# Qualcomm-AI-research/fastforward

Hardware: AMD Instinct MI355X
Metric: tokens/sec Llama-3-8B W8A8 quantized fwd; quant/dequant GB/s vs HBM peak (higher is better)
Workload: dtype int8; 1 GPU; llama3-8b shapes, W8 per-channel symmetric + A8 per-tensor asymmetric on the 7 linears x 32 layers (BASELINE.json configs[2] forward), weights re-quantized every step as in the reference; global_batch=8, seq_len=2048, parallelism=dp1 (batch-sharded replicas, no data-path collective), quantizers=448, launch=hipGraph replay

## Files before the change

### fastforward_amd/csrc/ffq_attention.hip

```cpp
#include "ffq_affine.h"
#include "ffq_common.h"
#include "ffq_vec.h"

#include <math.h>
#include <stdlib.h>


namespace ffq {
namespace {

typedef __attribute__((ext_vector_type(8))) __bf16 bf16x8;
typedef __attribute__((ext_vector_type(16))) float f32x16;
typedef __attribute__((ext_vector_type(4))) short s16x4;
typedef __attribute__((ext_vector_type(8))) short s16x8;

constexpr int kD = 128;
constexpr int kKeys = 64;
#ifndef FFQ_ATTN_WAVES
#define FFQ_ATTN_WAVES 8
#endif
constexpr int kWaves = FFQ_ATTN_WAVES;
constexpr int kRowsPerWave = 32;
constexpr int kQBlock = kWaves * kRowsPerWave;
constexpr int kKPitch = 256;
constexpr int kVPitch = 320;
constexpr int kKBytes = kKeys * kKPitch;
constexpr int kVBytes = kKeys * kVPitch;
constexpr int kLdsBytes = 2 * kKBytes + 2 * kVBytes;
constexpr float kDefer = 8.0f;
constexpr int kOPitch = 272;
static_assert(kWaves * kRowsPerWave * kOPitch <= kLdsBytes, "epilogue image must fit the K/V ring");

struct AttnArgs {
  const uint16_t* q;
  const uint16_t* k;
  const uint16_t* v;
  uint16_t* ctx;
  int8_t* codes;
  const float* scale;
  const float* offset;
  int32_t B, S, H, HKV;
  int32_t nqb;
  float c;
  float lo, hi;
  const uint16_t* q_cos;
  const uint16_t* q_sin;
};

__device__ __forceinline__ bf16x8 load_vt(const unsigned char* vbuf, uint32_t lane_off, int imm) {
  typedef s16x4 __attribute__((address_space(3))) * lds_ptr;
  const s16x4 a = __builtin_amdgcn_ds_read_tr16_b64_v4i16((lds_ptr)(vbuf + lane_off + imm));
  const s16x4 b = __builtin_amdgcn_ds_read_tr16_b64_v4i16((lds_ptr)(vbuf + lane_off + imm + 8 * kVPitch));
  const s16x8 ab = __builtin_shufflevector(a, b, 0, 1, 2, 3, 4, 5, 6, 7);
  return __builtin_bit_cast(bf16x8, ab);
}

template <bool CAUSAL>
__global__ __launch_bounds__(kWaves * 64) void attention_fwd_kernel(AttnArgs a) {
  constexpr int QBLOCK = kQBlock;
  constexpr int PASSES = kKeys / (kWaves * 4);

  extern __shared__ __attribute__((aligned(16))) unsigned char smem[];
  const uint32_t tid = threadIdx.x;
  const uint32_t lane = tid & 63, wave = tid >> 6;
  const uint32_t r32 = lane & 31, h = lane >> 5;

  const uint32_t groups = (uint32_t)(a.H / a.HKV);
  uint32_t bid = blockIdx.x;
  const uint32_t kvh = bid % (uint32_t)a.HKV;
  bid /= (uint32_t)a.HKV;
  const uint32_t hg = bid % groups;
  bid /= groups;
  const uint32_t qb = (uint32_t)a.nqb - 1 - bid % (uint32_t)a.nqb;
  const uint32_t b = bid / (uint32_t)a.nqb;
  const uint32_t head = kvh * groups + hg;

  const int32_t q0 = (int32_t)qb * QBLOCK;
  const int32_t qw0 = q0 + (int32_t)wave * kRowsPerWave;
  const bool wave_valid = qw0 < a.S;
  const int32_t q_end = q0 + QBLOCK < a.S ? q0 + QBLOCK : a.S;
  const int32_t ntiles = (CAUSAL ? q_end : a.S) / kKeys;

  const uint32_t srow = tid >> 4, sslot = tid & 15;
  const size_t kv_stride = (size_t)a.HKV * kD;
  const uint16_t* kbase = a.k + ((size_t)b * a.S * a.HKV + kvh) * kD + sslot * 8;
  const uint16_t* vbase = a.v + ((size_t)b * a.S * a.HKV + kvh) * kD + sslot * 8;
  u32x4 sk[PASSES], sv[PASSES];
  auto stage_load = [&](int32_t tile) {
#pragma unroll
    for (int p = 0; p < PASSES; ++p) {
      const size_t row = (size_t)tile * kKeys + srow + kWaves * 4 * p;
      sk[p] = *reinterpret_cast<const u32x4*>(kbase + row * kv_stride);
      sv[p] = *reinterpret_cast<const u32x4*>(vbase + row * kv_stride);
    }
  };
  auto stage_store = [&](int buf) {
#pragma unroll
    for (int p = 0; p < PASSES; ++p) {
      const uint32_t row = srow + kWaves * 4 * p;
      *reinterpret_cast<u32x4*>(smem + buf * kKBytes + row * kKPitch + ((sslot ^ (row & 15)) << 4)) = sk[p];
      *reinterpret_cast<u32x4*>(smem + 2 * kKBytes + buf * kVBytes + row * kVPitch + (sslot << 4)) = sv[p];
    }
  };

  stage_load(0);

  bf16x8 qf[8];
  {
    const uint16_t* qrow = a.q + (((size_t)b * a.S + (size_t)(wave_valid ? qw0 + (int32_t)r32 : 0)) * a.H + head) * kD;
#pragma unroll
    for (int t = 0; t < 8; ++t) {
      u32x4 v = *reinterpret_cast<const u32x4*>(qrow + (2 * t + h) * 8);
      if (!wave_valid) v = u32x4{0, 0, 0, 0};
      qf[t] = __builtin_bit_cast(bf16x8, v);
    }
    if (a.q_cos && wave_valid) {
      const size_t trow = (size_t)(qw0 + (int32_t)r32) * kD;
#pragma unroll
      for (int t = 0; t < 4; ++t) {
        const int c = (2 * t + (int)h) * 8;
        const u32x4 cl = *reinterpret_cast<const u32x4*>(a.q_cos + trow + c), ch = *reinterpret_cast<const u32x4*>(a.q_cos + trow + 64 + c);
        const u32x4 sl = *reinterpret_cast<const u32x4*>(a.q_sin + trow + c), sh = *reinterpret_cast<const u32x4*>(a.q_sin + trow + 64 + c);
        const u32x4 lo = __builtin_bit_cast(u32x4, qf[t]), hi = __builtin_bit_cast(u32x4, qf[t + 4]);
        const uint32_t lw[4] = {lo.x, lo.y, lo.z, lo.w}, hw[4] = {hi.x, hi.y, hi.z, hi.w};
        const uint32_t clw[4] = {cl.x, cl.y, cl.z, cl.w}, chw[4] = {ch.x, ch.y, ch.z, ch.w};
        const uint32_t slw[4] = {sl.x, sl.y, sl.z, sl.w}, shw[4] = {sh.x, sh.y, sh.z, sh.w};
        uint32_t ol[4], oh[4];
#pragma unroll
        for (int w = 0; w < 4; ++w) {
          float r[2][2];
#pragma unroll
          for (int e = 0; e < 2; ++e) {
            auto el = [&](uint32_t word) { return __builtin_bit_cast(float, e ? (word & 0xFFFF0000u) : (word << 16)); };
            const float x1 = el(lw[w]), x2 = el(hw[w]);
            float p = x1 * el(clw[w]), q2 = (-x2) * el(slw[w]), u = x2 * el(chw[w]), d = x1 * el(shw[w]);
            const uint32_t pq = pack2<bf16_t>(p, q2), ud = pack2<bf16_t>(u, d);
            r[0][e] = __builtin_bit_cast(float, pq << 16) + __builtin_bit_cast(float, pq & 0xFFFF0000u);
            r[1][e] = __builtin_bit_cast(float, ud << 16) + __builtin_bit_cast(float, ud & 0xFFFF0000u);
          }
          ol[w] = pack2<bf16_t>(r[0][0], r[0][1]);
          oh[w] = pack2<bf16_t>(r[1][0], r[1][1]);
        }
        qf[t] = __builtin_bit_cast(bf16x8, u32x4{ol[0], ol[1], ol[2], ol[3]});
        qf[t + 4] = __builtin_bit_cast(bf16x8, u32x4{oh[0], oh[1], oh[2], oh[3]});
      }
    }
  }

  f32x16 o[4];
#pragma unroll
  for (int i = 0; i < 4; ++i)
#pragma unroll
    for (int e = 0; e < 16; ++e) o[i][e] = 0.0f;
  float m_run = -1.0e30f, l_run = 0.0f;

  const uint32_t i16 = lane & 15, g16 = lane >> 4;
  const uint32_t vt_lane_off = (4 * (g16 >> 1) + (i16 >> 2)) * kVPitch + (16 * (g16 & 1) + 4 * (i16 & 3)) * 2;

  stage_store(0);
  __syncthreads();

  for (int32_t tile = 0; tile < ntiles; ++tile) {
    const int buf = tile & 1;
    const bool more = tile + 1 < ntiles;
    if (more) stage_load(tile + 1);
    const int32_t kv0 = tile * kKeys;
    const bool active = wave_valid && (!CAUSAL || kv0 <= qw0 + kRowsPerWave - 1);
    if (active) {
      const unsigned char* kbuf = smem + buf * kKBytes;
      const unsigned char* vbuf = smem + 2 * kKBytes + buf * kVBytes;
      f32x16 s[2];
#pragma unroll
      for (int sub = 0; sub < 2; ++sub)
#pragma unroll
        for (int e = 0; e < 16; ++e) s[sub][e] = 0.0f;
      bf16x8 kf[2][8];
#pragma unroll
      for (int t = 0; t < 8; ++t)
#pragma unroll
        for (int sub = 0; sub < 2; ++sub) {
          const uint32_t krow = 32 * sub + r32;
          kf[sub][t] = *reinterpret_cast<const bf16x8*>(kbuf + krow * kKPitch + (((2 * t + h) ^ (krow & 15)) << 4));
        }
#pragma unroll
      for (int t = 0; t < 8; ++t)
#pragma unroll
        for (int sub = 0; sub < 2; ++sub)
          s[sub] = __builtin_amdgcn_mfma_f32_32x32x16_bf16(kf[sub][t], qf[t], s[sub], 0, 0, 0);
      __builtin_amdgcn_sched_group_barrier(0x100, 16, 0);
      __builtin_amdgcn_sched_group_barrier(0x008, 16, 0);
      if (CAUSAL && kv0 + kKeys - 1 > qw0) {
        const int32_t qi = qw0 + (int32_t)r32;
#pragma unroll
        for (int sub = 0; sub < 2; ++sub)
#pragma unroll
          for (int e = 0; e < 16; ++e) {
            const int32_t key = kv0 + 32 * sub + (e & 3) + 8 * (e >> 2) + 4 * (int32_t)h;
            if (key > qi) s[sub][e] = -INFINITY;
          }
      }
      float mx = s[0][0];
#pragma unroll
      for (int sub = 0; sub < 2; ++sub)
#pragma unroll
        for (int e = 0; e < 16; ++e) mx = fmaxf(mx, s[sub][e]);
      mx = fmaxf(mx, __shfl_xor(mx, 32));
      const float mxs = mx * a.c;
      if (!__all(mxs - m_run <= kDefer)) {
        const float m_new = mxs - m_run > kDefer ? mxs : m_run;
        const float alpha = __builtin_amdgcn_exp2f(m_run - m_new);
        m_run = m_new;
        l_run *= alpha;
#pragma unroll
        for (int i = 0; i < 4; ++i)
#pragma unroll
          for (int e = 0; e < 16; ++e) o[i][e] *= alpha;
      }
      float rs = 0.0f;
      bf16x8 pf[2][2];
#pragma unroll
      for (int sub = 0; sub < 2; ++sub)
#pragma unroll
        for (int e = 0; e < 16; ++e) {
          const float p = __builtin_amdgcn_exp2f(__builtin_fmaf(s[sub][e], a.c, -m_run));
          rs += p;
          pf[sub][e >> 3][e & 7] = (__bf16)p;
        }
      l_run += rs;
#pragma unroll
      for (int db = 0; db < 4; ++db)
#pragma unroll
        for (int sub = 0; sub < 2; ++sub)
#pragma unroll
          for (int u = 0; u < 2; ++u) {
            const int imm = (32 * sub + 16 * u) * kVPitch + 32 * db * 2;
            const bf16x8 vf = load_vt(vbuf, vt_lane_off, imm);
            o[db] = __builtin_amdgcn_mfma_f32_32x32x16_bf16(vf, pf[sub][u], o[db], 0, 0, 0);
          }
    }
    if (more) stage_store(buf ^ 1);
    __syncthreads();
  }

  const float l_tot = l_run + __shfl_xor(l_run, 32);
  const float inv = 1.0f / l_tot;
  unsigned char* obuf = smem + wave * (kRowsPerWave * kOPitch);
#pragma unroll
  for (int db = 0; db < 4; ++db)
#pragma unroll
    for (int rr = 0; rr < 4; ++rr) {
      u32x2 w;
      w.x = pack2<bf16_t>(o[db][4 * rr + 0] * inv, o[db][4 * rr + 1] * inv);
      w.y = pack2<bf16_t>(o[db][4 * rr + 2] * inv, o[db][4 * rr + 3] * inv);
      *reinterpret_cast<u32x2*>(obuf + r32 * kOPitch + (32 * db + 8 * rr + 4 * h) * 2) = w;
    }
  __syncthreads();
  if (!wave_valid) return;
  float sc = 1.0f, of = 0.0f;
  if (a.codes) {
    sc = a.scale[0];
    of = a.offset ? rne(a.offset[0]) : 0.0f;
  }
#pragma unroll
  for (int it = 0; it < 4; ++it) {
    const uint32_t slot = it * 64 + lane;
    const uint32_t row = slot >> 3, seg = slot & 7;
    Chunk<bf16_t, 16> z;
    z.load(reinterpret_cast<const bf16_t*>(obuf + row * kOPitch + seg * 32));
    const size_t at = (((size_t)b * a.S + (size_t)(qw0 + (int32_t)row)) * a.H + head) * kD + seg * 16;
    if (a.ctx) z.store(reinterpret_cast<bf16_t*>(a.ctx) + at);
    if (a.codes) {
      float x[16];
#pragma unroll
      for (int i = 0; i < 16; ++i) x[i] = z.get(i);
      Chunk<int8_t, 16> y;
      quantize_chunk_to_bytes<16>(x, sc, of, a.lo, a.hi, y);
      y.store(a.codes + at);
    }
  }
}

}
}

using namespace ffq;

extern "C" int ffq_attention(const void* q, const void* k, const void* v, int dt, int64_t batch, int64_t seq_len,
                             int64_t q_heads, int64_t kv_heads, int64_t head_dim, double softmax_scale, int causal,
                             void* ctx_out, int8_t* codes_out, const float* out_scale, const float* out_offset,
                             double out_num_bits, const void* q_cos, const void* q_sin, void* stream) {
  hipStream_t s = static_cast<hipStream_t>(stream);
  if (batch < 0 || seq_len < 0 || q_heads <= 0 || kv_heads <= 0) return fail(FFQ_ERR_ARG, "bad extent");
  if (dt != FFQ_BF16) return fail(FFQ_ERR_DTYPE, "attention is built for bf16 activations");
  if (head_dim != kD) return fail(FFQ_ERR_DTYPE, "attention is built for head_dim 128");
  if (seq_len % kKeys != 0) return fail(FFQ_ERR_DTYPE, "attention needs seq_len %% 64 == 0");
  if (q_heads % kv_heads != 0) return fail(FFQ_ERR_ARG, "q_heads must be a multiple of kv_heads");
  if (batch == 0 || seq_len == 0) return FFQ_OK;
  if (!q || !k || !v || (!ctx_out && !codes_out)) return fail(FFQ_ERR_ARG, "NULL buffer");
  if (codes_out && !out_scale) return fail(FFQ_ERR_ARG, "codes need a scale");
  if (codes_out && !(out_num_bits >= 1.0 && out_num_bits <= 8.0 && out_num_bits == (double)(int)out_num_bits))
    return fail(FFQ_ERR_ARG, "codes need an integral bit-width in 1..8");
  if (!aligned16(q) || !aligned16(k) || !aligned16(v) || (ctx_out && !aligned16(ctx_out)) || (codes_out && !aligned16(codes_out)))
    return fail(FFQ_ERR_ARG, "buffers must be 16-byte aligned");
  if (batch * seq_len * q_heads * head_dim >= ((int64_t)1 << 40)) return fail(FFQ_ERR_ARG, "too many elements for one launch");
  if ((q_cos == nullptr) != (q_sin == nullptr)) return fail(FFQ_ERR_ARG, "q_cos and q_sin come together");
  if (q_cos && (!aligned16(q_cos) || !aligned16(q_sin))) return fail(FFQ_ERR_ARG, "buffers must be 16-byte aligned");
  AttnArgs a;
  a.q_cos = static_cast<const uint16_t*>(q_cos); a.q_sin = static_cast<const uint16_t*>(q_sin);
  a.q = static_cast<const uint16_t*>(q); a.k = static_cast<const uint16_t*>(k); a.v = static_cast<const uint16_t*>(v);
  a.ctx = static_cast<uint16_t*>(ctx_out); a.codes = codes_out; a.scale = out_scale; a.offset = out_offset;
  a.B = (int32_t)batch; a.S = (int32_t)seq_len; a.H = (int32_t)q_heads; a.HKV = (int32_t)kv_heads;
  a.nqb = (int32_t)((seq_len + kQBlock - 1) / kQBlock);
  a.c = (float)(softmax_scale * 1.4426950408889634);
  const double half = ldexp(1.0, (int)out_num_bits - 1);
  a.lo = codes_out ? (float)-half : 0.0f;
  a.hi = codes_out ? (float)(half - 1.0) : 0.0f;
  const int64_t blocks = (int64_t)a.nqb * q_heads * batch;
  if (blocks >= ((int64_t)1 << 31)) return fail(FFQ_ERR_ARG, "too many workgroups");
  static uint64_t once_causal = 0, once_full = 0;
  if (causal) ensure_dynamic_lds(&once_causal, reinterpret_cast<const void*>(attention_fwd_kernel<true>), kLdsBytes);
  else ensure_dynamic_lds(&once_full, reinterpret_cast<const void*>(attention_fwd_kernel<false>), kLdsBytes);
  const dim3 grid((unsigned)blocks), block(kWaves * 64);
  if (causal) attention_fwd_kernel<true><<<grid, block, kLdsBytes, s>>>(a);
  else attention_fwd_kernel<false><<<grid, block, kLdsBytes, s>>>(a);
  return check_launch("attention_fwd_kernel");
}
```

### fastforward_amd/csrc/ffq_common.h

```cpp
#pragma once

#include <hip/hip_runtime.h>
#include <stdarg.h>
#include <stdint.h>
#include <stdio.h>

#include "../../include/ffq.h"

#ifndef FFQ_TICKET_ORDER
#define FFQ_TICKET_ORDER __ATOMIC_RELAXED
#endif
#define ffq_ticket_acquire()                                                      \
  do {                                                                            \
    if (FFQ_TICKET_ORDER != __ATOMIC_RELAXED) __builtin_amdgcn_fence(__ATOMIC_ACQUIRE, "agent"); \
  } while (0)

namespace ffq {

char* err_buf();
int fail(int code, const char* fmt, ...);
bool generic_kernels_forced();
bool mid_register_form_forced();
bool splitk_abandon_forced();
bool ring3_form_forced();
bool two_slot_form_forced();
int check_launch(const char* what);

__host__ __device__ inline bool dt_valid(int dt) { return dt >= FFQ_F32 && dt <= FFQ_U8; }
__host__ __device__ inline bool dt_is_float(int dt) {
  return dt == FFQ_F32 || dt == FFQ_BF16 || dt == FFQ_F16 || dt == FFQ_F64;
}
__host__ __device__ inline int dt_size(int dt) {
  switch (dt) {
    case FFQ_F32: case FFQ_I32: return 4;
    case FFQ_BF16: case FFQ_F16: case FFQ_I16: return 2;
    case FFQ_F64: case FFQ_I64: return 8;
    default: return 1;
  }
}

__host__ __device__ inline float bf16_bits_to_f32(uint16_t h) {
  return __builtin_bit_cast(float, (uint32_t)h << 16);
}
__host__ __device__ inline uint16_t f32_to_bf16_bits(float f) {
  uint32_t u = __builtin_bit_cast(uint32_t, f);
  if (f != f) return 0x7FC0;
  u += 0x7FFFu + ((u >> 16) & 1u);
  return (uint16_t)(u >> 16);
}
__host__ __device__ inline float f16_bits_to_f32(uint16_t h) {
  return (float)__builtin_bit_cast(_Float16, h);
}
__host__ __device__ inline uint16_t f32_to_f16_bits(float f) {
  return __builtin_bit_cast(uint16_t, (_Float16)f);
}

__host__ __device__ inline float round_stage(float v, int dt) {
  if (dt == FFQ_BF16) return bf16_bits_to_f32(f32_to_bf16_bits(v));
  if (dt == FFQ_F16) return f16_bits_to_f32(f32_to_f16_bits(v));
  return v;
}

__host__ __device__ inline float rne(float v) { return __builtin_rintf(v); }
__host__ __device__ inline double rne(double v) { return __builtin_rint(v); }

__host__ __device__ inline float clamp_nan(float v, float lo, float hi) {
  float c = v < lo ? lo : v;
  c = c > hi ? hi : c;
  return v != v ? v : c;
}
__host__ __device__ inline double clamp_nan(double v, double lo, double hi) {
  double c = v < lo ? lo : v;
  c = c > hi ? hi : c;
  return v != v ? v : c;
}

__device__ inline double load_any(const void* p, int dt, int64_t i) {
  switch (dt) {
    case FFQ_F32: return (double)((const float*)p)[i];
    case FFQ_BF16: return (double)bf16_bits_to_f32(((const uint16_t*)p)[i]);
    case FFQ_F16: return (double)f16_bits_to_f32(((const uint16_t*)p)[i]);
    case FFQ_F64: return ((const double*)p)[i];
    case FFQ_I8: return (double)((const int8_t*)p)[i];
    case FFQ_I16: return (double)((const int16_t*)p)[i];
    case FFQ_I32: return (double)((const int32_t*)p)[i];
    case FFQ_I64: return (double)((const int64_t*)p)[i];
    default: return (double)((const uint8_t*)p)[i];
  }
}
__device__ inline void store_any(void* p, int dt, int64_t i, double v) {
  const bool nan = v != v;
  switch (dt) {
    case FFQ_F32: ((float*)p)[i] = (float)v; break;
    case FFQ_BF16: ((uint16_t*)p)[i] = f32_to_bf16_bits((float)v); break;
    case FFQ_F16: ((uint16_t*)p)[i] = f32_to_f16_bits((float)v); break;
    case FFQ_F64: ((double*)p)[i] = v; break;
    case FFQ_I8: ((int8_t*)p)[i] = nan ? 0 : (int8_t)(int64_t)v; break;
    case FFQ_I16: ((int16_t*)p)[i] = nan ? 0 : (int16_t)(int64_t)v; break;
    case FFQ_I32: ((int32_t*)p)[i] = nan ? INT32_MIN : (int32_t)(int64_t)v; break;
    case FFQ_I64: ((int64_t*)p)[i] = nan ? INT64_MIN : (int64_t)v; break;
    default: ((uint8_t*)p)[i] = nan ? 0 : (uint8_t)(int64_t)v; break;
  }
}

struct FastDiv {
  uint32_t mul;
  uint32_t shift;
  uint32_t div;
// ... 103 lines not shown
```

### fastforward_amd/csrc/ffq_core.hip

```cpp
#include "ffq_common.h"

#include <math.h>
#include <string.h>

namespace ffq {

static thread_local char g_err[512];

char* err_buf() { return g_err; }

int fail(int code, const char* fmt, ...) {
  va_list ap;
  va_start(ap, fmt);
  vsnprintf(g_err, sizeof g_err, fmt, ap);
  va_end(ap);
  return code;
}

int check_launch(const char* what) {
  hipError_t e = hipGetLastError();
  if (e != hipSuccess) return fail(FFQ_ERR_LAUNCH, "%s: %s", what, hipGetErrorString(e));
  return FFQ_OK;
}

// ... 87 lines not shown
              "The size of tensor a (%lld) must match the size of tensor b (%lld) at non-singleton "
              "dimension 0 (%s vs number of tiles)",
              (long long)ntiles, (long long)numel, what);
}

GenericTiling make_generic(const ffq_tiling* t) {
  GenericTiling g;
  memset(&g, 0, sizeof g);
  g.ndim = t->ndim;
  int64_t s = 1;
  for (int k = t->ndim - 1; k >= 0; --k) {
    g.shape[k] = t->shape[k];
    g.tile[k] = t->tile[k];
    g.gstride[k] = s;
    s *= t->shape[k] / t->tile[k];
  }
  return g;
}

}

using namespace ffq;

extern "C" {

int ffq_abi_version(void) { return FFQ_ABI_VERSION; }
const char* ffq_last_error(void) { return err_buf(); }
const char* ffq_backend_name(void) { return "hip:gfx950"; }

int64_t ffq_num_tiles(const ffq_tiling* tiling) {
  TileInfo info;
  int rc = analyse(tiling, &info);
  if (rc) return -rc;
  return info.ntiles;
}

int ffq_promote_types(int a, int b) {
  if (!dt_valid(a) || !dt_valid(b)) return -FFQ_ERR_ARG;
  if (a == b) return a;
  const bool fa = dt_is_float(a), fb = dt_is_float(b);
  if (fa && !fb) return a;
  if (fb && !fa) return b;
  if (fa && fb) {
    if (a == FFQ_F64 || b == FFQ_F64) return FFQ_F64;
    return FFQ_F32;
  }
  if (a == FFQ_I64 || b == FFQ_I64) return FFQ_I64;
  if (a == FFQ_I32 || b == FFQ_I32) return FFQ_I32;
  return FFQ_I16;
}

int ffq_can_support_bitwidth(int dtype, double num_bits) {
  double avail;
  switch (dtype) {
    case FFQ_BF16: avail = 7; break;
    case FFQ_F16: avail = 10; break;
    case FFQ_F32: avail = 23; break;
    case FFQ_F64: avail = 52; break;
    case FFQ_I8: case FFQ_U8: avail = 8; break;
    case FFQ_I16: avail = 16; break;
    case FFQ_I32: avail = 32; break;
    case FFQ_I64: avail = 64; break;
    default: return 0;
  }
  return (avail + 2) >= num_bits;
}

int ffq_dequantize_result_dtype(int data_dt, int scale_dt, int offset_dt, int has_offset) {
  const int off_dt = has_offset ? offset_dt : scale_dt;
  const int add_dt = ffq_promote_types(data_dt, off_dt);
  if (add_dt < 0) return add_dt;
  return ffq_promote_types(add_dt, scale_dt);
}

}

namespace ffq {
static int g_force_generic = 0;
bool generic_kernels_forced() { return (__atomic_load_n(&g_force_generic, __ATOMIC_RELAXED) & 1) != 0; }
bool splitk_abandon_forced() { return (__atomic_load_n(&g_force_generic, __ATOMIC_RELAXED) & 2) != 0; }
bool mid_register_form_forced() { return (__atomic_load_n(&g_force_generic, __ATOMIC_RELAXED) & 4) != 0; }
bool ring3_form_forced() { return (__atomic_load_n(&g_force_generic, __ATOMIC_RELAXED) & 8) != 0; }
bool two_slot_form_forced() { return (__atomic_load_n(&g_force_generic, __ATOMIC_RELAXED) & 16) != 0; }
}

extern "C" int ffq_force_generic_kernels(int on) {
  return __atomic_exchange_n(&ffq::g_force_generic, on & 31, __ATOMIC_RELAXED);
}
```

Baseline: 139,700 tokens/s.

## Replace per-block attention grid with persistent sorted work walk and GQA head packing

Attention now launches a persistent grid capped at 256 workgroups. Each workgroup walks a list of (batch, kv-head, head-group, row-block) items sorted by causal length and alternates direction on odd rounds, with an XCD-preserving mapping. When the GQA group size is 2, 4 or 8, the heads sharing one KV head are packed into a single item so K/V tiles are loaded once for several query heads. The next item's K/V and Q loads overlap the epilogue of the current one. The aim is to reduce causal tail imbalance and K/V refetch, at the cost of more complex scheduling and extra barriers; the old block form stays available behind a force flag.

```diff
diff --git a/fastforward_amd/csrc/ffq_attention.hip b/fastforward_amd/csrc/ffq_attention.hip
--- a/fastforward_amd/csrc/ffq_attention.hip
+++ b/fastforward_amd/csrc/ffq_attention.hip
@@ -1,4 +1,5 @@
 #include "ffq_affine.h"
+#include "ffq_attn_walk.h"
 #include "ffq_common.h"
 #include "ffq_vec.h"
 
@@ -19,9 +20,13 @@
 #ifndef FFQ_ATTN_WAVES
 #define FFQ_ATTN_WAVES 8
 #endif
+#ifndef FFQ_ATTN_PACK
+#define FFQ_ATTN_PACK 1
+#endif
 constexpr int kWaves = FFQ_ATTN_WAVES;
+constexpr int kAttnWalkWorkgroups = 256;
+static_assert(kWaves * 32 == kWalkBlockRows && 64 == kWalkKeys, "ffq_attn_walk.h describes 8 waves of 32 rows and 64-key tiles");
 constexpr int kRowsPerWave = 32;
-constexpr int kQBlock = kWaves * kRowsPerWave;
 constexpr int kKPitch = 256;
 constexpr int kVPitch = 320;
 constexpr int kKBytes = kKeys * kKPitch;
@@ -40,7 +45,6 @@
   const float* scale;
   const float* offset;
   int32_t B, S, H, HKV;
-  int32_t nqb;
   float c;
   float lo, hi;
   const uint16_t* q_cos;
@@ -55,219 +59,230 @@
   return __builtin_bit_cast(bf16x8, ab);
 }
 
+
+struct Lane {
+  uint32_t lane, wave, r32, h;
+  uint32_t srow, sslot;
+  uint32_t vt_lane_off;
+};
+
+__device__ __forceinline__ Lane make_lane(uint32_t tid, uint32_t wave) {
+  Lane ln;
+  ln.lane = tid & 63; ln.wave = wave;
+  ln.r32 = ln.lane & 31; ln.h = ln.lane >> 5;
+  ln.srow = tid >> 4; ln.sslot = tid & 15;
+  const uint32_t i16 = ln.lane & 15, g16 = ln.lane >> 4;
+  ln.vt_lane_off = (4 * (g16 >> 1) + (i16 >> 2)) * kVPitch + (16 * (g16 & 1) + 4 * (i16 & 3)) * 2;
+  return ln;
+}
+
+constexpr int kPasses = kKeys / (kWaves * 4);
+struct Stage {
+  u32x4 sk[kPasses], sv[kPasses];
+};
+
+
+__device__ __forceinline__ size_t kv_base(const AttnArgs& a, uint32_t b, uint32_t kvh) { return ((size_t)b * a.S * a.HKV + kvh) * kD; }
+
+__device__ __forceinline__ void stage_load(Stage& st, const AttnArgs& a, const Lane& ln, size_t base, int32_t tile) {
+  const uint32_t kv_stride = (uint32_t)a.HKV * kD;
+  const uint32_t lane_off = ln.srow * kv_stride + ln.sslot * 8;
+#pragma unroll
+  for (int p = 0; p < kPasses; ++p) {
+    const size_t rows = base + ((size_t)tile * kKeys + kWaves * 4 * p) * kv_stride;
+    st.sk[p] = *reinterpret_cast<const u32x4*>(a.k + rows + lane_off);
+    st.sv[p] = *reinterpret_cast<const u32x4*>(a.v + rows + lane_off);
+  }
+}
+
+__device__ __forceinline__ void stage_store(const Stage& st, unsigned char* smem, const Lane& ln, int buf) {
+#pragma unroll
+  for (int p = 0; p < kPasses; ++p) {
+    const uint32_t row = ln.srow + kWaves * 4 * p;
+    *reinterpret_cast<u32x4*>(smem + buf * kKBytes + row * kKPitch + ((ln.sslot ^ (row & 15)) << 4)) = st.sk[p];
+    *reinterpret_cast<u32x4*>(smem + 2 * kKBytes + buf * kVBytes + row * kVPitch + (ln.sslot << 4)) = st.sv[p];
+  }
+}
+
+__device__ __forceinline__ void load_q(const AttnArgs& a, const Lane& ln, uint32_t b, uint32_t head, int32_t qw0, bool wave_valid, bf16x8 (&qf)[8]) {
+  if (wave_valid) {
+    const uint16_t* qrows = a.q + (((size_t)b * a.S + (size_t)qw0) * a.H + head) * kD;
+    const uint32_t lane_off = ln.r32 * ((uint32_t)a.H * kD) + ln.h * 8;
+#pragma unroll
+    for (int t = 0; t < 8; ++t) qf[t] = __builtin_bit_cast(bf16x8, *reinterpret_cast<const u32x4*>(qrows + lane_off + 16 * t));
+  } else {
+#pragma unroll
+    for (int t = 0; t < 8; ++t) qf[t] = __builtin_bit_cast(bf16x8, u32x4{0, 0, 0, 0});
+  }
+}
+
+__device__ __forceinline__ void rotate_q(const AttnArgs& a, const Lane& ln, int32_t qw0, bf16x8 (&qf)[8]) {
+  const uint16_t* cos0 = a.q_cos + (size_t)qw0 * kD;
+  const uint16_t* sin0 = a.q_sin + (size_t)qw0 * kD;
+  const uint32_t lane_off = ln.r32 * kD + ln.h * 8;
+  u32x4 tcl[4], tch[4], tsl[4], tsh[4];
+#pragma unroll
+  for (int t = 0; t < 4; ++t) {
+    const uint32_t c = lane_off + 16 * t;
+    tcl[t] = *reinterpret_cast<const u32x4*>(cos0 + c); tch[t] = *reinterpret_cast<const u32x4*>(cos0 + c + 64);
+    tsl[t] = *reinterpret_cast<const u32x4*>(sin0 + c); tsh[t] = *reinterpret_cast<const u32x4*>(sin0 + c + 64);
+  }
+#pragma unroll
+  for (int t = 0; t < 4; ++t) {
+    const u32x4 cl = tcl[t], ch = tch[t], sl = tsl[t], sh = tsh[t];
+    const u32x4 lo = __builtin_bit_cast(u32x4, qf[t]), hi = __builtin_bit_cast(u32x4, qf[t + 4]);
+    const uint32_t lw[4] = {lo.x, lo.y, lo.z, lo.w}, hw[4] = {hi.x, hi.y, hi.z, hi.w};
+    const uint32_t clw[4] = {cl.x, cl.y, cl.z, cl.w}, chw[4] = {ch.x, ch.y, ch.z, ch.w};
+    const uint32_t slw[4] = {sl.x, sl.y, sl.z, sl.w}, shw[4] = {sh.x, sh.y, sh.z, sh.w};
+    uint32_t ol[4], oh[4];
+#pragma unroll
+    for (int w = 0; w < 4; ++w) {
+      float r[2][2];
+#pragma unroll
+      for (int e = 0; e < 2; ++e) {
+        auto el = [&](uint32_t word) { return __builtin_bit_cast(float, e ? (word & 0xFFFF0000u) : (word << 16)); };
+        const float x1 = el(lw[w]), x2 = el(hw[w]);
+        float p = x1 * el(clw[w]), q2 = (-x2) * el(slw[w]), u = x2 * el(chw[w]), d = x1 * el(shw[w]);
+        const uint32_t pq = pack2<bf16_t>(p, q2), ud = pack2<bf16_t>(u, d);
+        r[0][e] = __builtin_bit_cast(float, pq << 16) + __builtin_bit_cast(float, pq & 0xFFFF0000u);
+        r[1][e] = __builtin_bit_cast(float, ud << 16) + __builtin_bit_cast(float, ud & 0xFFFF0000u);
+      }
+      ol[w] = pack2<bf16_t>(r[0][0], r[0][1]);
+      oh[w] = pack2<bf16_t>(r[1][0], r[1][1]);
+    }
+    qf[t] = __builtin_bit_cast(bf16x8, u32x4{ol[0], ol[1], ol[2], ol[3]});
+    qf[t + 4] = __builtin_bit_cast(bf16x8, u32x4{oh[0], oh[1], oh[2], oh[3]});
+  }
+}
+
+struct RowState {
+  f32x16 o[4];
+  float m_run, l_run;
+};
+
+__device__ __forceinline__ void reset_rows(RowState& rs) {
+#pragma unroll
+  for (int i = 0; i < 4; ++i)
+#pragma unroll
+    for (int e = 0; e < 16; ++e) rs.o[i][e] = 0.0f;
+  rs.m_run = -1.0e30f;
+  rs.l_run = 0.0f;
+}
+
 template <bool CAUSAL>
-__global__ __launch_bounds__(kWaves * 64) void attention_fwd_kernel(AttnArgs a) {
-  constexpr int QBLOCK = kQBlock;
-  constexpr int PASSES = kKeys / (kWaves * 4);
-
-  extern __shared__ __attribute__((aligned(16))) unsigned char smem[];
-  const uint32_t tid = threadIdx.x;
-  const uint32_t lane = tid & 63, wave = tid >> 6;
-  const uint32_t r32 = lane & 31, h = lane >> 5;
-
-  const uint32_t groups = (uint32_t)(a.H / a.HKV);
-  uint32_t bid = blockIdx.x;
-  const uint32_t kvh = bid % (uint32_t)a.HKV;
-  bid /= (uint32_t)a.HKV;
-  const uint32_t hg = bid % groups;
-  bid /= groups;
-  const uint32_t qb = (uint32_t)a.nqb - 1 - bid % (uint32_t)a.nqb;
-  const uint32_t b = bid / (uint32_t)a.nqb;
-  const uint32_t head = kvh * groups + hg;
-
-  const int32_t q0 = (int32_t)qb * QBLOCK;
-  const int32_t qw0 = q0 + (int32_t)wave * kRowsPerWave;
-  const bool wave_valid = qw0 < a.S;
-  const int32_t q_end = q0 + QBLOCK < a.S ? q0 + QBLOCK : a.S;
-  const int32_t ntiles = (CAUSAL ? q_end : a.S) / kKeys;
-
-  const uint32_t srow = tid >> 4, sslot = tid & 15;
-  const size_t kv_stride = (size_t)a.HKV * kD;
-  const uint16_t* kbase = a.k + ((size_t)b * a.S * a.HKV + kvh) * kD + sslot * 8;
-  const uint16_t* vbase = a.v + ((size_t)b * a.S * a.HKV + kvh) * kD + sslot * 8;
-  u32x4 sk[PASSES], sv[PASSES];
-  auto stage_load = [&](int32_t tile) {
-#pragma unroll
-    for (int p = 0; p < PASSES; ++p) {
-      const size_t row = (size_t)tile * kKeys + srow + kWaves * 4 * p;
-      sk[p] = *reinterpret_cast<const u32x4*>(kbase + row * kv_stride);
-      sv[p] = *reinterpret_cast<const u32x4*>(vbase + row * kv_stride);
-    }
-  };
-  auto stage_store = [&](int buf) {
-#pragma unroll
-    for (int p = 0; p < PASSES; ++p) {
-      const uint32_t row = srow + kWaves * 4 * p;
-      *reinterpret_cast<u32x4*>(smem + buf * kKBytes + row * kKPitch + ((sslot ^ (row & 15)) << 4)) = sk[p];
-      *reinterpret_cast<u32x4*>(smem + 2 * kKBytes + buf * kVBytes + row * kVPitch + (sslot << 4)) = sv[p];
-    }
-  };
-
-  stage_load(0);
-
-  bf16x8 qf[8];
-  {
-    const uint16_t* qrow = a.q + (((size_t)b * a.S + (size_t)(wave_valid ? qw0 + (int32_t)r32 : 0)) * a.H + head) * kD;
-#pragma unroll
-    for (int t = 0; t < 8; ++t) {
-      u32x4 v = *reinterpret_cast<const u32x4*>(qrow + (2 * t + h) * 8);
-      if (!wave_valid) v = u32x4{0, 0, 0, 0};
-      qf[t] = __builtin_bit_cast(bf16x8, v);
-    }
-    if (a.q_cos && wave_valid) {
-      const size_t trow = (size_t)(qw0 + (int32_t)r32) * kD;
-#pragma unroll
-      for (int t = 0; t < 4; ++t) {
-        const int c = (2 * t + (int)h) * 8;
-        const u32x4 cl = *reinterpret_cast<const u32x4*>(a.q_cos + trow + c), ch = *reinterpret_cast<const u32x4*>(a.q_cos + trow + 64 + c);
-        const u32x4 sl = *reinterpret_cast<const u32x4*>(a.q_sin + trow + c), sh = *reinterpret_cast<const u32x4*>(a.q_sin + trow + 64 + c);
-        const u32x4 lo = __builtin_bit_cast(u32x4, qf[t]), hi = __builtin_bit_cast(u32x4, qf[t + 4]);
-        const uint32_t lw[4] = {lo.x, lo.y, lo.z, lo.w}, hw[4] = {hi.x, hi.y, hi.z, hi.w};
-        const uint32_t clw[4] = {cl.x, cl.y, cl.z, cl.w}, chw[4] = {ch.x, ch.y, ch.z, ch.w};
-        const uint32_t slw[4] = {sl.x, sl.y, sl.z, sl.w}, shw[4] = {sh.x, sh.y, sh.z, sh.w};
-        uint32_t ol[4], oh[4];
-#pragma unroll
-        for (int w = 0; w < 4; ++w) {
-          float r[2][2];
-#pragma unroll
-          for (int e = 0; e < 2; ++e) {
-            auto el = [&](uint32_t word) { return __builtin_bit_cast(float, e ? (word & 0xFFFF0000u) : (word << 16)); };
-            const float x1 = el(lw[w]), x2 = el(hw[w]);
-            float p = x1 * el(clw[w]), q2 = (-x2) * el(slw[w]), u = x2 * el(chw[w]), d = x1 * el(shw[w]);
-            const uint32_t pq = pack2<bf16_t>(p, q2), ud = pack2<bf16_t>(u, d);
-            r[0][e] = __builtin_bit_cast(float, pq << 16) + __builtin_bit_cast(float, pq & 0xFFFF0000u);
-            r[1][e] = __builtin_bit_cast(float, ud << 16) + __builtin_bit_cast(float, ud & 0xFFFF0000u);
-          }
-          ol[w] = pack2<bf16_t>(r[0][0], r[0][1]);
-          oh[w] = pack2<bf16_t>(r[1][0], r[1][1]);
-        }
-        qf[t] = __builtin_bit_cast(bf16x8, u32x4{ol[0], ol[1], ol[2], ol[3]});
-        qf[t + 4] = __builtin_bit_cast(bf16x8, u32x4{oh[0], oh[1], oh[2], oh[3]});
+__device__ __forceinline__ void tile_step(const AttnArgs& a, const Lane& ln, const unsigned char* kbuf, const unsigned char* vbuf, int32_t kv0,
+                                          int32_t qw0, const bf16x8 (&qf)[8], RowState& st) {
+  const uint32_t r32 = ln.r32, h = ln.h;
+  f32x16 (&o)[4] = st.o;
+  float& m_run = st.m_run;
+  float& l_run = st.l_run;
+  f32x16 s[2];
+#pragma unroll
+  for (int sub = 0; sub < 2; ++sub)
+#pragma unroll
+    for (int e = 0; e < 16; ++e) s[sub][e] = 0.0f;
+  bf16x8 kf[2][8];
+#pragma unroll
+  for (int t = 0; t < 8; ++t)
+#pragma unroll
+    for (int sub = 0; sub < 2; ++sub) {
+      const uint32_t krow = 32 * sub + r32;
+      kf[sub][t] = *reinterpret_cast<const bf16x8*>(kbuf + krow * kKPitch + (((2 * t + h) ^ (krow & 15)) << 4));
+    }
+#pragma unroll
+  for (int t = 0; t < 8; ++t)
+#pragma unroll
+    for (int sub = 0; sub < 2; ++sub)
+      s[sub] = __builtin_amdgcn_mfma_f32_32x32x16_bf16(kf[sub][t], qf[t], s[sub], 0, 0, 0);
+  __builtin_amdgcn_sched_group_barrier(0x100, 16, 0);
+  __builtin_amdgcn_sched_group_barrier(0x008, 16, 0);
+  if (CAUSAL && kv0 + kKeys - 1 > qw0) {
+    const int32_t qi = qw0 + (int32_t)r32;
+#pragma unroll
+    for (int sub = 0; sub < 2; ++sub)
+#pragma unroll
+      for (int e = 0; e < 16; ++e) {
+        const int32_t key = kv0 + 32 * sub + (e & 3) + 8 * (e >> 2) + 4 * (int32_t)h;
+        if (key > qi) s[sub][e] = -INFINITY;
       }
-    }
-  }
-
-  f32x16 o[4];
-#pragma unroll
-  for (int i = 0; i < 4; ++i)
-#pragma unroll
-    for (int e = 0; e < 16; ++e) o[i][e] = 0.0f;
-  float m_run = -1.0e30f, l_run = 0.0f;
-
-  const uint32_t i16 = lane & 15, g16 = lane >> 4;
-  const uint32_t vt_lane_off = (4 * (g16 >> 1) + (i16 >> 2)) * kVPitch + (16 * (g16 & 1) + 4 * (i16 & 3)) * 2;
-
-  stage_store(0);
-  __syncthreads();
-
-  for (int32_t tile = 0; tile < ntiles; ++tile) {
-    const int buf = tile & 1;
-    const bool more = tile + 1 < ntiles;
-    if (more) stage_load(tile + 1);
-    const int32_t kv0 = tile * kKeys;
-    const bool active = wave_valid && (!CAUSAL || kv0 <= qw0 + kRowsPerWave - 1);
-    if (active) {
-      const unsigned char* kbuf = smem + buf * kKBytes;
-      const unsigned char* vbuf = smem + 2 * kKBytes + buf * kVBytes;
-      f32x16 s[2];
-#pragma unroll
-      for (int sub = 0; sub < 2; ++sub)
-#pragma unroll
-        for (int e = 0; e < 16; ++e) s[sub][e] = 0.0f;
-      bf16x8 kf[2][8];
-#pragma unroll
-      for (int t = 0; t < 8; ++t)
-#pragma unroll
-        for (int sub = 0; sub < 2; ++sub) {
-          const uint32_t krow = 32 * sub + r32;
-          kf[sub][t] = *reinterpret_cast<const bf16x8*>(kbuf + krow * kKPitch + (((2 * t + h) ^ (krow & 15)) << 4));
-        }
-#pragma unroll
-      for (int t = 0; t < 8; ++t)
-#pragma unroll
-        for (int sub = 0; sub < 2; ++sub)
-          s[sub] = __builtin_amdgcn_mfma_f32_32x32x16_bf16(kf[sub][t], qf[t], s[sub], 0, 0, 0);
-      __builtin_amdgcn_sched_group_barrier(0x100, 16, 0);
-      __builtin_amdgcn_sched_group_barrier(0x008, 16, 0);
-      if (CAUSAL && kv0 + kKeys - 1 > qw0) {
-        const int32_t qi = qw0 + (int32_t)r32;
-#pragma unroll
-        for (int sub = 0; sub < 2; ++sub)
-#pragma unroll
-          for (int e = 0; e < 16; ++e) {
-            const int32_t key = kv0 + 32 * sub + (e & 3) + 8 * (e >> 2) + 4 * (int32_t)h;
-            if (key > qi) s[sub][e] = -INFINITY;
-          }
+  }
+  float mx = s[0][0];
+#pragma unroll
+  for (int sub = 0; sub < 2; ++sub)
+#pragma unroll
+    for (int e = 0; e < 16; ++e) mx = fmaxf(mx, s[sub][e]);
+  mx = fmaxf(mx, __shfl_xor(mx, 32));
+  const float mxs = mx * a.c;
+  if (!__all(mxs - m_run <= kDefer)) {
+    const float m_new = mxs - m_run > kDefer ? mxs : m_run;
+    const float alpha = __builtin_amdgcn_exp2f(m_run - m_new);
+    m_run = m_new;
+    l_run *= alpha;
+#pragma unroll
+    for (int i = 0; i < 4; ++i)
+#pragma unroll
+      for (int e = 0; e < 16; ++e) o[i][e] *= alpha;
+  }
+  float rs = 0.0f;
+  bf16x8 pf[2][2];
+#pragma unroll
+  for (int sub = 0; sub < 2; ++sub)
+#pragma unroll
+    for (int e = 0; e < 16; ++e) {
+      const float p = __builtin_amdgcn_exp2f(__builtin_fmaf(s[sub][e], a.c, -m_run));
+      rs += p;
+      pf[sub][e >> 3][e & 7] = (__bf16)p;
+    }
+  l_run += rs;
+#pragma unroll
+  for (int db = 0; db < 4; ++db)
+#pragma unroll
+    for (int sub = 0; sub < 2; ++sub)
+#pragma unroll
+      for (int u = 0; u < 2; ++u) {
+        const int imm = (32 * sub + 16 * u) * kVPitch + 32 * db * 2;
+        const bf16x8 vf = load_vt(vbuf, ln.vt_lane_off, imm);
+        o[db] = __builtin_amdgcn_mfma_f32_32x32x16_bf16(vf, pf[sub][u], o[db], 0, 0, 0);
       }
-      float mx = s[0][0];
-#pragma unroll
-      for (int sub = 0; sub < 2; ++sub)
-#pragma unroll
-        for (int e = 0; e < 16; ++e) mx = fmaxf(mx, s[sub][e]);
-      mx = fmaxf(mx, __shfl_xor(mx, 32));
-      const float mxs = mx * a.c;
-      if (!__all(mxs - m_run <= kDefer)) {
-        const float m_new = mxs - m_run > kDefer ? mxs : m_run;
-        const float alpha = __builtin_amdgcn_exp2f(m_run - m_new);
-        m_run = m_new;
-        l_run *= alpha;
-#pragma unroll
-        for (int i = 0; i < 4; ++i)
-#pragma unroll
-          for (int e = 0; e < 16; ++e) o[i][e] *= alpha;
-      }
-      float rs = 0.0f;
-      bf16x8 pf[2][2];
-#pragma unroll
-      for (int sub = 0; sub < 2; ++sub)
-#pragma unroll
-        for (int e = 0; e < 16; ++e) {
-          const float p = __builtin_amdgcn_exp2f(__builtin_fmaf(s[sub][e], a.c, -m_run));
-          rs += p;
-          pf[sub][e >> 3][e & 7] = (__bf16)p;
-        }
-      l_run += rs;
-#pragma unroll
-      for (int db = 0; db < 4; ++db)
-#pragma unroll
-        for (int sub = 0; sub < 2; ++sub)
-#pragma unroll
-          for (int u = 0; u < 2; ++u) {
-            const int imm = (32 * sub + 16 * u) * kVPitch + 32 * db * 2;
-            const bf16x8 vf = load_vt(vbuf, vt_lane_off, imm);
-            o[db] = __builtin_amdgcn_mfma_f32_32x32x16_bf16(vf, pf[sub][u], o[db], 0, 0, 0);
-          }
-    }
-    if (more) stage_store(buf ^ 1);
-    __syncthreads();
-  }
-
-  const float l_tot = l_run + __shfl_xor(l_run, 32);
+}
+
+__device__ __forceinline__ void epilogue_image(const RowState& st, const Lane& ln, unsigned char* obuf) {
+  const float l_tot = st.l_run + __shfl_xor(st.l_run, 32);
   const float inv = 1.0f / l_tot;
-  unsigned char* obuf = smem + wave * (kRowsPerWave * kOPitch);
 #pragma unroll
   for (int db = 0; db < 4; ++db)
 #pragma unroll
     for (int rr = 0; rr < 4; ++rr) {
       u32x2 w;
-      w.x = pack2<bf16_t>(o[db][4 * rr + 0] * inv, o[db][4 * rr + 1] * inv);
-      w.y = pack2<bf16_t>(o[db][4 * rr + 2] * inv, o[db][4 * rr + 3] * inv);
-      *reinterpret_cast<u32x2*>(obuf + r32 * kOPitch + (32 * db + 8 * rr + 4 * h) * 2) = w;
-    }
-  __syncthreads();
-  if (!wave_valid) return;
-  float sc = 1.0f, of = 0.0f;
+      w.x = pack2<bf16_t>(st.o[db][4 * rr + 0] * inv, st.o[db][4 * rr + 1] * inv);
+      w.y = pack2<bf16_t>(st.o[db][4 * rr + 2] * inv, st.o[db][4 * rr + 3] * inv);
+      *reinterpret_cast<u32x2*>(obuf + ln.r32 * kOPitch + (32 * db + 8 * rr + 4 * ln.h) * 2) = w;
+    }
+}
+
+struct CodeParams {
+  float sc, of;
+};
+
+__device__ __forceinline__ CodeParams code_params(const AttnArgs& a) {
+  CodeParams cp{1.0f, 0.0f};
   if (a.codes) {
-    sc = a.scale[0];
-    of = a.offset ? rne(a.offset[0]) : 0.0f;
-  }
+    cp.sc = a.scale[0];
+    cp.of = a.offset ? rne(a.offset[0]) : 0.0f;
+  }
+  return cp;
+}
+
+__device__ __forceinline__ void epilogue_rows(const AttnArgs& a, const Lane& ln, const unsigned char* obuf, uint32_t b, uint32_t head, int32_t qw0,
+                                              const CodeParams& cp) {
+  const float sc = cp.sc, of = cp.of;
 #pragma unroll
   for (int it = 0; it < 4; ++it) {
-    const uint32_t slot = it * 64 + lane;
+    const uint32_t slot = it * 64 + ln.lane;
     const uint32_t row = slot >> 3, seg = slot & 7;
     Chunk<bf16_t, 16> z;
     z.load(reinterpret_cast<const bf16_t*>(obuf + row * kOPitch + seg * 32));
-    const size_t at = (((size_t)b * a.S + (size_t)(qw0 + (int32_t)row)) * a.H + head) * kD + seg * 16;
+    const size_t at = (((size_t)b * a.S + (size_t)qw0) * a.H + head) * kD + (row * ((uint32_t)a.H * kD) + seg * 16);
     if (a.ctx) z.store(reinterpret_cast<bf16_t*>(a.ctx) + at);
     if (a.codes) {
       float x[16];
@@ -277,6 +292,127 @@
       quantize_chunk_to_bytes<16>(x, sc, of, a.lo, a.hi, y);
       y.store(a.codes + at);
     }
+  }
+}
+
+template <bool CAUSAL>
+__global__ __launch_bounds__(kWaves * 64) void attention_fwd_kernel(AttnArgs a, AttnWalk wk) {
+  extern __shared__ __attribute__((aligned(16))) unsigned char smem[];
+  const Lane ln = make_lane(threadIdx.x, threadIdx.x >> 6);
+  const AttnItem it = attn_block_item(wk, blockIdx.x);
+  uint32_t head;
+  int32_t qw0;
+  attn_wave_rows(wk, it, ln.wave, &head, &qw0);
+  const bool wave_valid = qw0 < a.S;
+  const size_t kvb = kv_base(a, it.b, it.kvh);
+
+  Stage sg;
+  stage_load(sg, a, ln, kvb, 0);
+  bf16x8 qf[8];
+  load_q(a, ln, it.b, head, qw0, wave_valid, qf);
+  if (a.q_cos && wave_valid) rotate_q(a, ln, qw0, qf);
+  RowState st;
+  reset_rows(st);
+  stage_store(sg, smem, ln, 0);
+  __syncthreads();
+
+  for (int32_t tile = 0; tile < it.ntiles; ++tile) {
+    const int buf = tile & 1;
+    const bool more = tile + 1 < it.ntiles;
+    if (more) stage_load(sg, a, ln, kvb, tile + 1);
+    const int32_t kv0 = tile * kKeys;
+    const bool active = wave_valid && (!CAUSAL || kv0 <= qw0 + kRowsPerWave - 1);
+    if (active) tile_step<CAUSAL>(a, ln, smem + buf * kKBytes, smem + 2 * kKBytes + buf * kVBytes, kv0, qw0, qf, st);
+    if (more) stage_store(sg, smem, ln, buf ^ 1);
+    __syncthreads();
+  }
+
+  unsigned char* obuf = smem + ln.wave * (kRowsPerWave * kOPitch);
+  epilogue_image(st, ln, obuf);
+  __syncthreads();
+  if (!wave_valid) return;
+  epilogue_rows(a, ln, obuf, it.b, head, qw0, code_params(a));
+}
+
+__device__ __forceinline__ Lane fresh_lane(uint32_t wave) {
+  uint32_t tid = threadIdx.x;
+  asm volatile("" : "+v"(tid));
+  return make_lane(tid, wave);
+}
+
+template <bool CAUSAL>
+__global__ __launch_bounds__(kWaves * 64) void attention_walk_kernel(AttnArgs a, AttnWalk wk) {
+  extern __shared__ __attribute__((aligned(16))) unsigned char smem[];
+  const uint32_t wave = (uint32_t)__builtin_amdgcn_readfirstlane((int)(threadIdx.x >> 6));
+  unsigned char* obuf = smem + wave * (kRowsPerWave * kOPitch);
+  CodeParams cp = code_params(a);
+  cp.sc = __builtin_bit_cast(float, __builtin_amdgcn_readfirstlane(__builtin_bit_cast(int, cp.sc)));
+  cp.of = __builtin_bit_cast(float, __builtin_amdgcn_readfirstlane(__builtin_bit_cast(int, cp.of)));
+
+  AttnItem it;
+  attn_walk_item(wk, blockIdx.x, 0, &it);
+  uint32_t head;
+  int32_t qw0;
+  attn_wave_rows(wk, it, wave, &head, &qw0);
+  bool wave_valid = qw0 < a.S;
+  size_t kvb = kv_base(a, it.b, it.kvh);
+
+  Stage sg;
+  bf16x8 qf[8];
+  {
+    const Lane ln = fresh_lane(wave);
+    stage_load(sg, a, ln, kvb, 0);
+    load_q(a, ln, it.b, head, qw0, wave_valid, qf);
+    if (a.q_cos && wave_valid) rotate_q(a, ln, qw0, qf);
+    stage_store(sg, smem, ln, 0);
+  }
+  __syncthreads();
+
+  for (uint32_t round = 1;; ++round) {
+    AttnItem nx = it;
+    const bool has_next = attn_walk_item(wk, blockIdx.x, round, &nx);
+    uint32_t nhead;
+    int32_t nqw0;
+    attn_wave_rows(wk, nx, wave, &nhead, &nqw0);
+    const bool nvalid = nqw0 < a.S;
+    const size_t nkvb = kv_base(a, nx.b, nx.kvh);
+
+    RowState st;
+    reset_rows(st);
+    {
+      const Lane ln = make_lane(threadIdx.x, wave);
+      const int32_t last = it.ntiles - 1;
+      for (int32_t tile = 0; tile < last; ++tile) {
+        const int buf = tile & 1;
+        stage_load(sg, a, ln, kvb, tile + 1);
+        const int32_t kv0 = tile * kKeys;
+        const bool active = wave_valid && (!CAUSAL || kv0 <= qw0 + kRowsPerWave - 1);
+        if (active) tile_step<CAUSAL>(a, ln, smem + buf * kKBytes, smem + 2 * kKBytes + buf * kVBytes, kv0, qw0, qf, st);
+        stage_store(sg, smem, ln, buf ^ 1);
+        __syncthreads();
+      }
+      const int buf = last & 1;
+      const int32_t kv0 = last * kKeys;
+      const bool active = wave_valid && (!CAUSAL || kv0 <= qw0 + kRowsPerWave - 1);
+      if (active) tile_step<CAUSAL>(a, ln, smem + buf * kKBytes, smem + 2 * kKBytes + buf * kVBytes, kv0, qw0, qf, st);
+    }
+    const Lane ln = fresh_lane(wave);
+    if (has_next) {
+      stage_load(sg, a, ln, nkvb, 0);
+      load_q(a, ln, nx.b, nhead, nqw0, nvalid, qf);
+    }
+    __syncthreads();
+
+    epilogue_image(st, ln, obuf);
+    __syncthreads();
+    if (has_next && a.q_cos && nvalid) rotate_q(a, ln, nqw0, qf);
+    __builtin_amdgcn_s_waitcnt(0x0F70);
+    if (wave_valid) epilogue_rows(a, ln, obuf, it.b, head, qw0, cp);
+    if (!has_next) break;
+    __syncthreads();
+    stage_store(sg, smem, ln, 0);
+    __syncthreads();
+    it = nx; head = nhead; qw0 = nqw0; wave_valid = nvalid; kvb = nkvb;
   }
 }
 
@@ -303,6 +439,7 @@
   if (!aligned16(q) || !aligned16(k) || !aligned16(v) || (ctx_out && !aligned16(ctx_out)) || (codes_out && !aligned16(codes_out)))
     return fail(FFQ_ERR_ARG, "buffers must be 16-byte aligned");
   if (batch * seq_len * q_heads * head_dim >= ((int64_t)1 << 40)) return fail(FFQ_ERR_ARG, "too many elements for one launch");
+  if (q_heads >= ((int64_t)1 << 16)) return fail(FFQ_ERR_ARG, "too many heads for one launch");
   if ((q_cos == nullptr) != (q_sin == nullptr)) return fail(FFQ_ERR_ARG, "q_cos and q_sin come together");
   if (q_cos && (!aligned16(q_cos) || !aligned16(q_sin))) return fail(FFQ_ERR_ARG, "buffers must be 16-byte aligned");
   AttnArgs a;
@@ -310,18 +447,26 @@
   a.q = static_cast<const uint16_t*>(q); a.k = static_cast<const uint16_t*>(k); a.v = static_cast<const uint16_t*>(v);
   a.ctx = static_cast<uint16_t*>(ctx_out); a.codes = codes_out; a.scale = out_scale; a.offset = out_offset;
   a.B = (int32_t)batch; a.S = (int32_t)seq_len; a.H = (int32_t)q_heads; a.HKV = (int32_t)kv_heads;
-  a.nqb = (int32_t)((seq_len + kQBlock - 1) / kQBlock);
   a.c = (float)(softmax_scale * 1.4426950408889634);
   const double half = ldexp(1.0, (int)out_num_bits - 1);
   a.lo = codes_out ? (float)-half : 0.0f;
   a.hi = codes_out ? (float)(half - 1.0) : 0.0f;
-  const int64_t blocks = (int64_t)a.nqb * q_heads * batch;
-  if (blocks >= ((int64_t)1 << 31)) return fail(FFQ_ERR_ARG, "too many workgroups");
-  static uint64_t once_causal = 0, once_full = 0;
-  if (causal) ensure_dynamic_lds(&once_causal, reinterpret_cast<const void*>(attention_fwd_kernel<true>), kLdsBytes);
-  else ensure_dynamic_lds(&once_full, reinterpret_cast<const void*>(attention_fwd_kernel<false>), kLdsBytes);
-  const dim3 grid((unsigned)blocks), block(kWaves * 64);
-  if (causal) attention_fwd_kernel<true><<<grid, block, kLdsBytes, s>>>(a);
-  else attention_fwd_kernel<false><<<grid, block, kLdsBytes, s>>>(a);
-  return check_launch("attention_fwd_kernel");
-}
+  if (batch * q_heads * ((seq_len + kRowsPerWave - 1) / kRowsPerWave) >= ((int64_t)1 << 31)) return fail(FFQ_ERR_ARG, "too many workgroups");
+  const dim3 block(kWaves * 64);
+  if (attention_block_form_forced()) {
+    const AttnWalk wk = attn_walk_make(batch, seq_len, q_heads, kv_heads, causal != 0, false, kAttnWalkWorkgroups);
+    static uint64_t once_causal = 0, once_full = 0;
+    if (causal) ensure_dynamic_lds(&once_causal, reinterpret_cast<const void*>(attention_fwd_kernel<true>), kLdsBytes);
+    else ensure_dynamic_lds(&once_full, reinterpret_cast<const void*>(attention_fwd_kernel<false>), kLdsBytes);
+    if (causal) attention_fwd_kernel<true><<<dim3(wk.items), block, kLdsBytes, s>>>(a, wk);
+    else attention_fwd_kernel<false><<<dim3(wk.items), block, kLdsBytes, s>>>(a, wk);
+    return check_launch("attention_fwd_kernel");
+  }
+  const AttnWalk wk = attn_walk_make(batch, seq_len, q_heads, kv_heads, causal != 0, FFQ_ATTN_PACK != 0, kAttnWalkWorkgroups);
+  static uint64_t walk_causal = 0, walk_full = 0;
+  if (causal) ensure_dynamic_lds(&walk_causal, reinterpret_cast<const void*>(attention_walk_kernel<true>), kLdsBytes);
+  else ensure_dynamic_lds(&walk_full, reinterpret_cast<const void*>(attention_walk_kernel<false>), kLdsBytes);
+  if (causal) attention_walk_kernel<true><<<dim3(wk.wgs), block, kLdsBytes, s>>>(a, wk);
+  else attention_walk_kernel<false><<<dim3(wk.wgs), block, kLdsBytes, s>>>(a, wk);
+  return check_launch("attention_walk_kernel");
+}
diff --git a/fastforward_amd/csrc/ffq_attn_walk.h b/fastforward_amd/csrc/ffq_attn_walk.h
--- /dev/null
+++ b/fastforward_amd/csrc/ffq_attn_walk.h
@@ -0,0 +1,97 @@
+#pragma once
+
+#include <stdint.h>
+
+#if defined(__HIPCC__)
+#define FFQ_WALK_FN __host__ __device__ inline
+#else
+#define FFQ_WALK_FN inline
+#endif
+
+namespace ffq {
+
+constexpr int32_t kWalkBlockRows = 256;
+constexpr int32_t kWalkWaveRows = 32;
+constexpr int32_t kWalkKeys = 64;
+
+struct AttnWalk {
+  int32_t B, S, H, HKV;
+  int32_t causal;
+  int32_t hpi;
+  int32_t rows;
+  int32_t nrb;
+  int32_t nhg;
+  uint32_t items;
+  uint32_t wgs;
+  int32_t keep_xcd;
+};
+
+struct AttnItem {
+  uint32_t b, kvh;
+  uint32_t head0;
+  int32_t r0;
+  int32_t ntiles;
+};
+
+FFQ_WALK_FN bool attn_walk_packs(int64_t groups) { return groups == 2 || groups == 4 || groups == 8; }
+
+FFQ_WALK_FN AttnWalk attn_walk_make(int64_t B, int64_t S, int64_t H, int64_t HKV, bool causal, bool packed, int64_t compute_units) {
+  AttnWalk w;
+  w.B = (int32_t)B; w.S = (int32_t)S; w.H = (int32_t)H; w.HKV = (int32_t)HKV;
+  w.causal = causal ? 1 : 0;
+  const int64_t g = H / HKV;
+  w.hpi = packed && attn_walk_packs(g) ? (int32_t)g : 1;
+  w.rows = kWalkBlockRows / w.hpi;
+  w.nrb = (int32_t)((S + w.rows - 1) / w.rows);
+  w.nhg = (int32_t)(g / w.hpi);
+  const int64_t items = B * HKV * w.nhg * w.nrb;
+  w.items = (uint32_t)items;
+  w.wgs = (uint32_t)(items < compute_units ? items : compute_units);
+  w.keep_xcd = (HKV % 8 == 0 && w.wgs % 8 == 0) ? 1 : 0;
+  return w;
+}
+
+FFQ_WALK_FN int32_t attn_item_tiles(const AttnWalk& w, int32_t r0) {
+  if (!w.causal) return w.S / kWalkKeys;
+  const int32_t end = r0 + w.rows < w.S ? r0 + w.rows : w.S;
+  return (end - 1) / kWalkKeys + 1;
+}
+
+FFQ_WALK_FN AttnItem attn_sorted_item(const AttnWalk& w, uint32_t j) {
+  AttnItem it;
+  it.kvh = j % (uint32_t)w.HKV; j /= (uint32_t)w.HKV;
+  const uint32_t hg = j % (uint32_t)w.nhg; j /= (uint32_t)w.nhg;
+  it.b = j % (uint32_t)w.B; j /= (uint32_t)w.B;
+  it.head0 = it.kvh * (uint32_t)(w.nhg * w.hpi) + hg * (uint32_t)w.hpi;
+  it.r0 = (w.nrb - 1 - (int32_t)j) * w.rows;
+  it.ntiles = attn_item_tiles(w, it.r0);
+  return it;
+}
+
+FFQ_WALK_FN bool attn_walk_item(const AttnWalk& w, uint32_t wg, uint32_t round, AttnItem* it) {
+  uint32_t slot = wg;
+  if (round & 1) slot = w.keep_xcd ? (w.wgs - 8 - (wg & ~7u)) + (wg & 7u) : w.wgs - 1 - wg;
+  const uint64_t j = (uint64_t)round * w.wgs + slot;
+  if (j >= w.items) return false;
+  *it = attn_sorted_item(w, (uint32_t)j);
+  return true;
+}
+
+FFQ_WALK_FN AttnItem attn_block_item(const AttnWalk& w, uint32_t bid) {
+  AttnItem it;
+  it.kvh = bid % (uint32_t)w.HKV; bid /= (uint32_t)w.HKV;
+  const uint32_t hg = bid % (uint32_t)w.nhg; bid /= (uint32_t)w.nhg;
+  it.head0 = it.kvh * (uint32_t)w.nhg + hg;
+  it.r0 = (w.nrb - 1 - (int32_t)(bid % (uint32_t)w.nrb)) * w.rows;
+  it.b = bid / (uint32_t)w.nrb;
+  it.ntiles = attn_item_tiles(w, it.r0);
+  return it;
+}
+
+FFQ_WALK_FN void attn_wave_rows(const AttnWalk& w, const AttnItem& it, uint32_t wave, uint32_t* head, int32_t* qw0) {
+  const uint32_t wph = (uint32_t)(kWalkBlockRows / kWalkWaveRows / w.hpi);
+  *head = it.head0 + wave / wph;
+  *qw0 = it.r0 + (int32_t)(wave % wph) * kWalkWaveRows;
+}
+
+}
diff --git a/fastforward_amd/csrc/ffq_common.h b/fastforward_amd/csrc/ffq_common.h
--- a/fastforward_amd/csrc/ffq_common.h
+++ b/fastforward_amd/csrc/ffq_common.h
@@ -24,6 +24,7 @@
 bool splitk_abandon_forced();
 bool ring3_form_forced();
 bool two_slot_form_forced();
+bool attention_block_form_forced();
 int check_launch(const char* what);
 
 __host__ __device__ inline bool dt_valid(int dt) { return dt >= FFQ_F32 && dt <= FFQ_U8; }
diff --git a/fastforward_amd/csrc/ffq_core.hip b/fastforward_amd/csrc/ffq_core.hip
--- a/fastforward_amd/csrc/ffq_core.hip
+++ b/fastforward_amd/csrc/ffq_core.hip
@@ -193,8 +193,9 @@
 bool mid_register_form_forced() { return (__atomic_load_n(&g_force_generic, __ATOMIC_RELAXED) & 4) != 0; }
 bool ring3_form_forced() { return (__atomic_load_n(&g_force_generic, __ATOMIC_RELAXED) & 8) != 0; }
 bool two_slot_form_forced() { return (__atomic_load_n(&g_force_generic, __ATOMIC_RELAXED) & 16) != 0; }
+bool attention_block_form_forced() { return (__atomic_load_n(&g_force_generic, __ATOMIC_RELAXED) & 32) != 0; }
 }
 
 extern "C" int ffq_force_generic_kernels(int on) {
-  return __atomic_exchange_n(&ffq::g_force_generic, on & 31, __ATOMIC_RELAXED);
-}
+  return __atomic_exchange_n(&ffq::g_force_generic, on & 63, __ATOMIC_RELAXED);
+}
```

Result: no change. 140,700 tokens/s (median of 6 runs) (+0.8%).
